# HMCL-UNIST/AD_MPC

Measured on AMD Instinct MI355X. Metric: MPC solves/sec (N=20, nx=7, nu=2, fp64), higher is better.
Workload: dtype f64

## Files before the change

ad_mpc_amd/csrc/admpc_fused20.hip:

```cpp
#include <hip/hip_runtime.h>
#include <type_traits>
#include <stdint.h>
#include <math.h>
#include "../../include/admpc.h"

namespace {

typedef double d4 __attribute__((ext_vector_type(4)));

#include "cond_common.h"

#if defined(ADMPC_PHASE_TIMERS) || defined(ADMPC_F20_TRACE)
__device__ unsigned long long g_f20_trace[4 * 8192];
#define F20_TRACE_BEGIN() const unsigned long long tr_t0 = clock_real(); unsigned long long tr_t1 = 0
#define F20_TRACE_MID() tr_t1 = clock_real()
#define F20_TRACE_END(inst) do { if (threadIdx.x == 0 && (inst) < 8192) { g_f20_trace[4 * (inst)] = tr_t0; g_f20_trace[4 * (inst) + 1] = clock_real(); g_f20_trace[4 * (inst) + 2] = blockIdx.x; g_f20_trace[4 * (inst) + 3] = tr_t1; } } while (0)
#else
#define F20_TRACE_BEGIN() do { } while (0)
#define F20_TRACE_MID() do { } while (0)
#define F20_TRACE_END(inst) do { } while (0)
#endif
#ifdef ADMPC_PHASE_TIMERS
__device__ unsigned long long g_f20_ticks[16];
#define F20_DECL() unsigned long long ph_acc[8] = {0, 0, 0, 0, 0, 0, 0, 0}; const unsigned long long ph_t0 = clock_ticks(); unsigned long long ph_last = ph_t0
// ... 43 lines not shown
    extern __shared__ double lds_raw[];
    double* const Hp = lds_raw + FusedLds::oH;
    double* const Lp = lds_raw + FusedLds::oL;
    double* const park = lds_raw + FusedLds::oPark;
    double* const cb = lds_raw + FusedLds::oCb;
    double* const invd = cb + 64;
    double* const sb = invd + 64;
    double* const sb2 = sb + 64;
    double* const JT = lds_raw + FusedLds::oJT;
    double* const GT = lds_raw + FusedLds::oGT;
    double* const bl = lds_raw + FusedLds::oBl;
    double* const dqC = lds_raw + FusedLds::oDqC;
    double* const gam = lds_raw + FusedLds::oGam;
    double* const dqE = lds_raw + FusedLds::oDqC;
    double* const dus = lds_raw + FusedLds::oGam;
    double* const slot = slotbuf + (size_t)blockIdx.x * FusedLds::NTRI;
    constexpr int slot_aux = 16;
#define PK_DL   park[0 * 64 + lane]
#define PK_DUU  park[1 * 64 + lane]
#define PK_G0   park[2 * 64 + lane]
#define PK_DDL  park[3 * 64 + lane]
#define PK_DDU  park[4 * 64 + lane]

    const Dense40Lds W{Hp, Lp, cb, invd};
    auto factorise = [&](const double dbar_, const double sodd_, const int lz_) __attribute__((always_inline)) {
        dense40_factorise(W, lz_, dbar_, sodd_, lz_, [&](double (&)[n]) __attribute__((always_inline)) {
            if (lz_ < n) Lp[lz_ * (lz_ + 1) / 2 + lz_] = 0.0;
        });
    };

    F20_DECL();
    bool first_ticket = true;
    int* const sch_incl = reinterpret_cast<int*>(lds_raw + FusedLds::oSch);
    int* const sch_cnt = sch_incl + 64;
    if (cap != 0) {
        LAUNDER_LANE(lane_s);
        const int c = sched[F20_BINS0 + F20_NB - 1 - lane_s];
        sch_cnt[lane_s] = c;
        sch_incl[lane_s] = wave_scan_incl_int(c);
        WSYNC();
    }
    auto ticket_entry_addr = [&](const int t, const int lane_) __attribute__((always_inline)) -> const int* {
        const int incl = sch_incl[lane_], c = sch_cnt[lane_];
        const unsigned long long m = __ballot(incl > t);
        if (m == 0ull) return nullptr;
        const int l = __ffsll((long long)m) - 1;
        const int base = __builtin_amdgcn_readlane(incl - c, l);
        return sched + F20_HDR + (size_t)(F20_NB - 1 - l) * cap + (t - base);
    };
    int next_inst = -2;
    const int grid = (int)gridDim.x;
// ... 265 lines not shown
            const int itmax = cf->ipm_iter_max;
            const bool try_unc = cf->ipm_try_unconstrained != 0.0;
            const double thw = cf->ipm_warm_thr, wrest = cf->ipm_warm_restart;
            const int fbit = (int)cf->ipm_fallback_iter;
            const double inv_nineq = 1.0 / (double)(8 * N + 2 * (N - 1));
            const double ubar_i = ubg[sc];
            const double dl_i = cf->lbu[ji] - ubar_i, duu_i = cf->ubu[ji] - ubar_i;
            double t[4], lam[4], sl = thr, su = thr;
            {
                const double r0[4] = { thr - dl_i, thr + duu_i, thr, thr };
#pragma unroll
                for (int i = 0; i < 4; ++i) { t[i] = r0[i] > thr ? r0[i] : thr; lam[i] = mu0 * rcp_nr(t[i]); }
            }
            double Dt[2] = {1.0, 1.0}, Dlam[2] = {0.0, 0.0}, Ddl = 0.0, Ddu = 0.0, dx6 = 0.0;
            if (dact) {
                const double x6 = xbg[lane * 7 + 6];
                Ddl = cf->lbx_delta - x6; Ddu = cf->ubx_delta - x6;
                dx6 = xh6_own;
                const double r0[2] = { dx6 - Ddl, Ddu - dx6 };
#pragma unroll
                for (int i = 0; i < 2; ++i) { Dt[i] = r0[i] > thr ? r0[i] : thr; Dlam[i] = mu0 * rcp_nr(Dt[i]); }
            }
            PK_DL = dl_i; PK_DUU = duu_i; PK_G0 = g0; PK_DDL = Ddl; PK_DDU = Ddu;
            WSYNC();

            double rmax_prev = 0.0, step = 1e300, stp_local = 1e300, alpha_prev = 1.0;
            bool solved = false, warmed = false, cons = false;
            if (try_unc) {
                int lt = lane; asm volatile("" : "+v"(lt));
                factorise(uact ? Rj : 1.0, 0.0, lt);
                const double xt = dense40_solve(W, uact ? -g0 : 0.0, lt);
                const double duc = uact ? xt : 0.0;
                cb[lane] = duc;
                WSYNC();
                const double du1_stage = lane < N ? cb[2 * lane + 1] : 0.0;
                const double pre = wave_scan_incl<OpSum>(du1_stage);
                const double dx6c = xh6_own + h * (pre - du1_stage);
                const bool ok = (!uact || (duc >= dl_i && duc <= duu_i)) && (!dact || (dx6c >= Ddl && dx6c <= Ddu));
                WSYNC();
                if (__all(ok)) { du = duc; solved = true; }
                else if (thw > 0.0) {
                    warmed = true;
                    du = duc;
                    sl = fmax(dl_i - duc, 0.0) + thw; su = fmax(duc - duu_i, 0.0) + thw;
                    const double r0[4] = { duc + sl - dl_i, su + duu_i - duc, sl, su };
#pragma unroll
                    for (int i = 0; i < 4; ++i) { t[i] = r0[i] > thw ? r0[i] : thw; lam[i] = mu0 * rcp_nr(t[i]); }
                    if (dact) {
                        dx6 = dx6c;
                        const double q0[2] = { dx6 - Ddl, Ddu - dx6 };
#pragma unroll
                        for (int i = 0; i < 2; ++i) { Dt[i] = q0[i] > thw ? q0[i] : thw; Dlam[i] = mu0 * rcp_nr(Dt[i]); }
                    }
                }
// ... 8 lines not shown
                const double q0[2] = { dx6 - PK_DDL, PK_DDU - dx6 };
#pragma unroll
                for (int i = 0; i < 2; ++i) { Dt[i] = dact ? (q0[i] > thr ? q0[i] : thr) : 1.0; Dlam[i] = dact ? mu0 * rcp_nr(Dt[i]) : 0.0; }
                alpha_prev = 1.0; stp_local = 1e300;
            };
        F20_STAMP(4);
            F20_TRACE_MID();
            if (!solved && try_unc) {
                asm volatile("s_waitcnt vmcnt(0)" ::: "memory");
                slot_fetch<FusedLds::NTRI, slot_aux>(Hp, slot, lane);
            }
            if (!solved)
            for (; it < itmax + (cons ? fbit : 0); ++it) {
                if (it == 0) __builtin_amdgcn_s_setprio(1);
                if (it == 2) __builtin_amdgcn_s_setprio(2);
                if (it == 4) __builtin_amdgcn_s_setprio(3);
                int lz = lane;
                asm volatile("" : "+v"(lz));
                const int trz = lz * (lz + 1) / 2;
                const bool uz = lz < n;
                double ru, mu, Dbar, S_i;
                {
                    double musum = 0.0, cmax = 0.0, rmax = 0.0;
                    double G0, G1, G2, G3;
                    {
                        const double i0 = rcp_nr(t[0]), i1 = rcp_nr(t[1]), i2_ = rcp_nr(t[2]), i3 = rcp_nr(t[3]);
                        G0 = lam[0] * i0; G1 = lam[1] * i1; G2 = lam[2] * i2_; G3 = lam[3] * i3;
                    }
#pragma unroll
                    for (int i = 0; i < 4; ++i) { const double rci = t[i] * lam[i]; musum += uact ? rci : 0.0; cmax = fmax(cmax, uact ? rci : 0.0); }
#pragma unroll
                    for (int i = 0; i < 2; ++i) { const double rci = Dt[i] * Dlam[i]; musum += dact ? rci : 0.0; cmax = fmax(cmax, dact ? rci : 0.0); }
                    const double G56 = Dlam[0] * rcp_nr(Dt[0]) + Dlam[1] * rcp_nr(Dt[1]);
                    Dbar = uact ? Rj + G0 * G2 * rcp_nr(G0 + G2) + G1 * G3 * rcp_nr(G1 + G3) : 1.0;
                    cb[lane] = uact ? du : 0.0;
                    const double dlam_pref = wave_scan_incl<OpSum>(dact ? (Dlam[1] - Dlam[0]) : 0.0);
                    sb[lane] = rdlane(dlam_pref, 63) - dlam_pref;
                    const double Ssuf_incl = wave_scan_incl<OpSum>(dact ? G56 : 0.0);
                    sb2[lane] = rdlane(Ssuf_incl, 63) - Ssuf_incl;
                    asm volatile("s_waitcnt vmcnt(0)" ::: "memory");
                    WSYNC();
                    double hdu = 0.0;
                    {
                        double Rd3[3];
#pragma unroll
                        for (int m = 0; m < 3; ++m) Rd3[m] = cb[16 * m + (lane & 15)];
                        double hv[n];
                        sym_row_40(hv, lds_byte_addr(Hp + (uz ? trz : 0)), lds_byte_addr(Hp + (uz ? lz : 0)));
                        static_for<0, n>([&](auto cc) __attribute__((always_inline)) {
                            constexpr int c = decltype(cc)::value;
                            fmac_rowbc_ld<c % 16>(hdu, Rd3[c / 16], hv[c]);
                        });
                    }
                    ru = hdu + Rj * du + PK_G0 - lam[0] + lam[1] + (ji ? h * sb[uact ? ki : 0] : 0.0);
                    S_i = h * h * sb2[uact ? ki : 0];
                    {
                        const double rd0 = du + sl - PK_DL - t[0], rd1 = -du + su + PK_DUU - t[1], rd2 = sl - t[2], rd3 = su - t[3];
                        const double rsl = rho_l - lam[0] - lam[2], rsu = rho_u - lam[1] - lam[3];
                        const double Drd0 = dx6 - PK_DDL - Dt[0], Drd1 = PK_DDU - dx6 - Dt[1];
                        double ra = OpMaxNan::f(fabs(ru), fabs(rsl)); ra = OpMaxNan::f(ra, fabs(rsu));
                        ra = OpMaxNan::f(ra, fabs(rd0)); ra = OpMaxNan::f(ra, fabs(rd1)); ra = OpMaxNan::f(ra, fabs(rd2)); ra = OpMaxNan::f(ra, fabs(rd3));
                        const double rb = OpMaxNan::f(fabs(Drd0), fabs(Drd1));
                        rmax = OpMaxNan::f(uact ? ra : 0.0, dact ? rb : 0.0);
                    }
                    mu = wave_reduce<OpSum>(musum) * inv_nineq;
                    cmax = wave_reduce<OpMax0>(cmax);
                    rmax = wave_reduce<OpMaxNan0>(rmax);
                    step = wave_reduce<OpMax0>(stp_local);
                    if (!(mu == mu) || !(rmax == rmax)) { failed = true; break; }
                    if (cmax <= tol_comp && step <= tol_step &&
                        (rmax <= tol_res || (it > 0 && rmax > 0.1 * rmax_prev && rmax <= ADMPC_IPM_FLOOR_CAP * tol_res))) break;
                    rmax_prev = rmax;
                }
                if (fbit > 0 && !cons && it >= fbit) {
                    cons = true; warmed = false;
                    cold_start();
                    rmax_prev = 0.0;
                    --it;
                    continue;
                }
                factorise(Dbar, (uz && ji) ? S_i : 0.0, lz);
#pragma unroll
                for (int i = 0; i < 4; ++i) asm volatile("" : "+v"(t[i]), "+v"(lam[i]));
#pragma unroll
                for (int i = 0; i < 2; ++i) asm volatile("" : "+v"(Dt[i]), "+v"(Dlam[i]));
                double it_[4], il_[4], rc[4], Dit[2], Dil[2], Drc[2];
#pragma unroll
                for (int i = 0; i < 4; ++i) { it_[i] = rcp_nr(t[i]); il_[i] = rcp_nr(lam[i]); rc[i] = t[i] * lam[i]; }
#pragma unroll
                for (int i = 0; i < 2; ++i) { Dit[i] = rcp_nr(Dt[i]); Dil[i] = rcp_nr(Dlam[i]); Drc[i] = Dt[i] * Dlam[i]; }
                const double G0 = lam[0] * it_[0], G1 = lam[1] * it_[1], G2 = lam[2] * it_[2], G3 = lam[3] * it_[3];
                const double iG02 = rcp_nr(G0 + G2), iG13 = rcp_nr(G1 + G3);
                const double G5 = Dlam[0] * Dit[0], G6 = Dlam[1] * Dit[1];
                const double rd0 = du + sl - PK_DL - t[0], rd1 = -du + su + PK_DUU - t[1], rd2 = sl - t[2], rd3 = su - t[3];
                const double rsl = rho_l - lam[0] - lam[2], rsu = rho_u - lam[1] - lam[3];
                const double Drd0 = dx6 - PK_DDL - Dt[0], Drd1 = PK_DDU - dx6 - Dt[1];

                double mu_aff = 0.0, dsl = 0.0, dsu = 0.0, ddu = 0.0, dt[4], dlam[4], Ddt[2], Ddlam[2];
#pragma unroll 1
                for (int pass = 0; pass < 2; ++pass) {
                    const double c0 = rc[0] * it_[0], c1 = rc[1] * it_[1], c2 = rc[2] * it_[2], c3 = rc[3] * it_[3];
                    const double e1 = rsl + c0 + c2 + G0 * rd0 + G2 * rd2;
                    const double e2 = rsu + c1 + c3 + G1 * rd1 + G3 * rd3;
                    const double etal = c0 + G0 * rd0 - G0 * e1 * iG02;
                    const double etau = -c1 - G1 * rd1 + G1 * e2 * iG13;
                    const double ek = dact ? (Drc[0] * Dit[0] + G5 * Drd0) - (Drc[1] * Dit[1] + G6 * Drd1) : 0.0;
                    const double epref = wave_scan_incl<OpSum>(ek);
                    sb[lane] = rdlane(epref, 63) - epref;
                    WSYNC();
                    double y = uact ? -(ru + etal + etau + (ji ? h * sb[ki] : 0.0)) : 0.0;
                    const double x = dense40_solve(W, y, lz);
                    if (pass == 1) slot_fetch<FusedLds::NTRI, slot_aux>(Hp, slot, lz);
                    ddu = uact ? x : 0.0;
                    cb[lane] = ddu;
                    WSYNC();
                    const double du1_stage = lane < N ? cb[2 * lane + 1] : 0.0;
                    const double pre = wave_scan_incl<OpSum>(du1_stage);
                    const double ddx6 = h * (pre - du1_stage);
                    dsl = -(e1 + G0 * ddu) * iG02;
                    dsu = -(e2 - G1 * ddu) * iG13;
                    dt[0] = ddu + dsl + rd0; dt[1] = -ddu + dsu + rd1; dt[2] = dsl + rd2; dt[3] = dsu + rd3;
                    const double Gs[4] = { G0, G1, G2, G3 };
                    double rr = 0.0;
#pragma unroll
                    for (int i = 0; i < 4; ++i) {
                        dlam[i] = -rc[i] * it_[i] - Gs[i] * dt[i];
                        rr = fmax(rr, uact ? fmax(-dt[i] * it_[i], -dlam[i] * il_[i]) : 0.0);
                    }
                    Ddt[0] = ddx6 + Drd0;  Ddlam[0] = -Drc[0] * Dit[0] - G5 * Ddt[0];
                    Ddt[1] = -ddx6 + Drd1; Ddlam[1] = -Drc[1] * Dit[1] - G6 * Ddt[1];
#pragma unroll
                    for (int i = 0; i < 2; ++i) rr = fmax(rr, dact ? fmax(-Ddt[i] * Dit[i], -Ddlam[i] * Dil[i]) : 0.0);
                    rr = wave_reduce<OpMax0>(rr);
                    const double amax = rr > 1.0 ? rcp_nr(rr) : 1.0;
// ... 225 lines not shown
```

ad_mpc_amd/csrc/dense40.h:

```cpp
#pragma once

__device__ __forceinline__ double rdlane(double v, int l) {
    int lo = __builtin_amdgcn_readlane(__double2loint(v), l);
    int hi = __builtin_amdgcn_readlane(__double2hiint(v), l);
    return __hiloint2double(hi, lo);
}

template <int CTRL, int ROW_MASK>
__device__ __forceinline__ double dpp_mov(double ident, double v) {
    int lo = __builtin_amdgcn_update_dpp(__double2loint(ident), __double2loint(v), CTRL, ROW_MASK, 0xf, false);
    int hi = __builtin_amdgcn_update_dpp(__double2hiint(ident), __double2hiint(v), CTRL, ROW_MASK, 0xf, false);
    return __hiloint2double(hi, lo);
}
template <int CTRL, bool ZF>
__device__ __forceinline__ double dpp_shr(double ident, double v) {
    if constexpr (ZF) {
        int lo = __builtin_amdgcn_update_dpp(0, __double2loint(v), CTRL, 0xf, 0xf, true);
        int hi = __builtin_amdgcn_update_dpp(0, __double2hiint(v), CTRL, 0xf, 0xf, true);
        return __hiloint2double(hi, lo);
    } else return dpp_mov<CTRL, 0xf>(ident, v);
}
struct OpSum { static constexpr bool zf = true; static __device__ __forceinline__ double id() { return 0.0; } static __device__ __forceinline__ double f(double a, double b) { return a + b; } };
struct OpMax { static constexpr bool zf = false; static __device__ __forceinline__ double id() { return -INFINITY; } static __device__ __forceinline__ double f(double a, double b) { return fmax(a, b); } };
struct OpMaxNan { static constexpr bool zf = false; static __device__ __forceinline__ double id() { return -INFINITY; }
// ... 15 lines not shown
#ifdef ADMPC_WSYNC_FENCE_ONLY
#define WSYNC() do { __builtin_amdgcn_fence(__ATOMIC_RELEASE, "wavefront"); __builtin_amdgcn_wave_barrier(); __builtin_amdgcn_fence(__ATOMIC_ACQUIRE, "wavefront"); } while (0)
#else
#define WSYNC() __syncthreads()
#endif

#include "subst_asm.inc"
__device__ __forceinline__ unsigned lds_byte_addr(const double* p) {
    return (unsigned)(size_t)(__attribute__((address_space(3))) const double*)p;
}
__device__ __forceinline__ void fwd_subst_40(double& y, const unsigned row_addr, const unsigned pub_addr) {
    asm volatile(ADMPC_FWD_SUBST_ASM_40 : "+{v[100:101]}"(y) : "{v102}"(row_addr), "{v103}"(pub_addr) : ADMPC_SUBST_CLOBBERS);
}
__device__ __forceinline__ void bwd_subst_40(double& x, const unsigned col_addr, const unsigned pub_addr) {
    asm volatile(ADMPC_BWD_SUBST_ASM_40 : "+{v[100:101]}"(x) : "{v102}"(col_addr), "{v103}"(pub_addr) : ADMPC_SUBST_CLOBBERS);
}

#define RB_OUT(a, o) "=&v"(a[o + 0]), "=&v"(a[o + 1]), "=&v"(a[o + 2]), "=&v"(a[o + 3]), "=&v"(a[o + 4]), "=&v"(a[o + 5]), "=&v"(a[o + 6]), \
                     "=&v"(a[o + 7]), "=&v"(a[o + 8]), "=&v"(a[o + 9]), "=&v"(a[o + 10]), "=&v"(a[o + 11]), "=&v"(a[o + 12]), "=&v"(a[o + 13]), \
                     "=&v"(a[o + 14]), "=&v"(a[o + 15]), "=&v"(a[o + 16]), "=&v"(a[o + 17]), "=&v"(a[o + 18]), "=&v"(a[o + 19])
__device__ __forceinline__ void newton_row_40(double (&a)[40], const unsigned row_addr, const double dbar, const double s_odd) {
    asm volatile(ADMPC_ROWBUILD_ASM_40_A : RB_OUT(a, 0) : "v"(row_addr), "v"(dbar), "v"(s_odd) : "s46", "s47", "memory");
    asm volatile(ADMPC_ROWBUILD_ASM_40_B : RB_OUT(a, 20) : "v"(row_addr), "v"(dbar), "v"(s_odd) : "s46", "s47", "memory");
}

__device__ __forceinline__ void sym_row_40(double (&a)[40], const unsigned row_addr, const unsigned col_addr) {
    asm volatile(ADMPC_SYMROW_ASM_40_A : RB_OUT(a, 0) : "v"(row_addr), "v"(col_addr) : "memory");
    asm volatile(ADMPC_SYMROW_ASM_40_B : RB_OUT(a, 20) : "v"(row_addr), "v"(col_addr) : "memory");
}
template <int NR>
__device__ __forceinline__ void newton_row_40_b(double (&a)[40], const unsigned row_addr, const double dbar, const double s_odd) {
    static_assert(NR == 47 || NR == 54, "generated variants");
    if constexpr (NR == 47) {
        asm volatile(ADMPC_ROWBUILD_ASM_40_A_R47 : RB_OUT(a, 0) : "v"(row_addr), "v"(dbar), "v"(s_odd) : "s46", "s47", "memory");
        asm volatile(ADMPC_ROWBUILD_ASM_40_B_R47 : RB_OUT(a, 20) : "v"(row_addr), "v"(dbar), "v"(s_odd) : "s46", "s47", "memory");
    } else {
        asm volatile(ADMPC_ROWBUILD_ASM_40_A_R54 : RB_OUT(a, 0) : "v"(row_addr), "v"(dbar), "v"(s_odd) : "s46", "s47", "memory");
        asm volatile(ADMPC_ROWBUILD_ASM_40_B_R54 : RB_OUT(a, 20) : "v"(row_addr), "v"(dbar), "v"(s_odd) : "s46", "s47", "memory");
    }
}
template <int NR>
__device__ __forceinline__ void sym_row_40_b(double (&a)[40], const unsigned row_addr, const unsigned col_addr) {
    if constexpr (NR == 47) {
        asm volatile(ADMPC_SYMROW_ASM_40_A_R47 : RB_OUT(a, 0) : "v"(row_addr), "v"(col_addr) : "memory");
        asm volatile(ADMPC_SYMROW_ASM_40_B_R47 : RB_OUT(a, 20) : "v"(row_addr), "v"(col_addr) : "memory");
    } else {
// ... 78 lines not shown
    const auto phi = __builtin_amdgcn_permlane16_swap(hi, hi, false, false);
    if (FIRST_ROW <= 0 || LAST_ROW >= 2) {
        const auto elo = __builtin_amdgcn_permlane32_swap(plo[0], plo[0], false, false);
        const auto ehi = __builtin_amdgcn_permlane32_swap(phi[0], phi[0], false, false);
        if (FIRST_ROW <= 0) R[0] = __hiloint2double((int)ehi[0], (int)elo[0]);
        if (LAST_ROW >= 2) R[2] = __hiloint2double((int)ehi[1], (int)elo[1]);
    }
    if (FIRST_ROW <= 1 && LAST_ROW >= 1) {
        const auto olo = __builtin_amdgcn_permlane32_swap(plo[1], plo[1], false, false);
        const auto ohi = __builtin_amdgcn_permlane32_swap(phi[1], phi[1], false, false);
        R[1] = __hiloint2double((int)ohi[0], (int)olo[0]);
    }
}

__device__ __forceinline__ double rcp_nr(double d) {
    double r = __builtin_amdgcn_rcp(d);
    double e = fma(-d, r, 1.0);
    r = fma(r, e, r);
    e = fma(-d, r, 1.0);
    return fma(r, e, r);
}


struct Dense40Lds { double *Hp, *Lp, *cb, *invd; };
struct Dense40NoFix { __device__ __forceinline__ void operator()(double (&)[40]) const {} };

template <class Fix = Dense40NoFix>
__device__ __forceinline__ void dense40_factorise(const Dense40Lds& W, const int lane, const double dbar_, const double sodd_, const int lz_, const Fix& fix = Fix())
{
    constexpr int n = 40;
    const int trz_ = lz_ * (lz_ + 1) / 2;
    const bool uz_ = lz_ < n;
    double a[n];
    newton_row_40(a, lds_byte_addr(W.Hp + (uz_ ? trz_ : 0)), dbar_, sodd_);
    fix(a);
    const unsigned lrow = lds_byte_addr(W.Lp + (uz_ ? trz_ : 0));
    const unsigned pub_wr = lds_byte_addr(W.cb + lane), pub_rd = lds_byte_addr(W.cb + (lane & 15));
    double* const invd = W.invd;
    auto chain = [&](auto jc, double& nln) __attribute__((always_inline)) {
        constexpr int j = decltype(jc)::value;
        const double dj = rdlane(a[j], j);
        const double dinv = rcp_nr(dj);
        const double lu = a[j] * dinv;
        invd[j] = dinv;
        if constexpr (j + 1 < n) {
            asm volatile("s_bfm_b64 exec, %2, %3\n\tds_write_b64 %0, %1 offset:%4\n\ts_mov_b64 exec, -1"
                         : : "v"(lrow), "v"(lu), "n"(n - 1 - j), "n"(j + 1), "n"(8 * j) : "memory");
            nln = -lu;
        }
    };
    double Rb[2][3] = {{0.0, 0.0, 0.0}, {0.0, 0.0, 0.0}}, nlb[2] = {0.0, 0.0};
    W.cb[lane] = a[0];
#pragma unroll
    for (int m = 0; m < 3; ++m) Rb[0][m] = W.cb[16 * m + (lane & 15)];
    chain(std::integral_constant<int, 0>{}, nlb[0]);
    static_for<0, n - 1>([&](auto jc) __attribute__((always_inline)) {
        constexpr int j = decltype(jc)::value;
        constexpr bool own = (j + 1) / 16 == 2;
        constexpr bool pub = j + 2 < n && (j + 2) / 16 < 2;
        double (&R)[3] = Rb[j & 1];
        double (&Rn)[3] = Rb[(j + 1) & 1];
        double& nl = nlb[j & 1];
        double& nln = nlb[(j + 1) & 1];
        col_head<j + 1, (j + 2) / 16, pub, own>(a[j + 1], R, nl, Rn, pub_wr, pub_rd);
        if constexpr (!pub) Rn[2] = a[j + 1];
        chain(std::integral_constant<int, j + 1>{}, nln);
        constexpr int j4 = ((j + 2 + 3) / 4) * 4 < n ? ((j + 2 + 3) / 4) * 4 : n;
        static_for<j + 2, j4>([&](auto c) __attribute__((always_inline)) {
            constexpr int jj = decltype(c)::value;
            if constexpr (own) fmac_rowbc<jj % 16>(a[jj], R[jj / 16], nl);
            else fmac_rowbc_ld<jj % 16>(a[jj], R[jj / 16], nl);
        });
        static_for<j4 / 4, n / 4>([&](auto c) __attribute__((always_inline)) {
            constexpr int jj = 4 * decltype(c)::value;
            if constexpr (own) fmac_rowbc4<jj % 16>(a[jj], a[jj + 1], a[jj + 2], a[jj + 3], R[jj / 16], nl);
            else fmac_rowbc4_ld<jj % 16>(a[jj], a[jj + 1], a[jj + 2], a[jj + 3], R[jj / 16], nl);
        });
    });
    WSYNC();
}

__device__ __forceinline__ double dense40_solve(const Dense40Lds& W, double y, const int lz_)
{
    const bool uz_ = lz_ < 40;
    const unsigned pub = lds_byte_addr(W.cb + (lz_ & 15));
    fwd_subst_40(y, lds_byte_addr(W.Lp + (uz_ ? lz_ * (lz_ + 1) / 2 : 0)), pub);
    double x = y * W.invd[uz_ ? lz_ : 0];
    bwd_subst_40(x, lds_byte_addr(W.Lp + (uz_ ? lz_ : 0)), pub);
    return x;
}

__device__ __forceinline__ double dense40_symv(const Dense40Lds& W, const int lane, const double v, const int lz_)
{
    constexpr int n = 40;
    const bool uz_ = lz_ < n;
    W.cb[lane] = v;
    WSYNC();
    double Rd3[3];
#pragma unroll
    for (int m = 0; m < 3; ++m) Rd3[m] = W.cb[16 * m + (lane & 15)];
    double hv[n];
    sym_row_40(hv, lds_byte_addr(W.Hp + (uz_ ? lz_ * (lz_ + 1) / 2 : 0)), lds_byte_addr(W.Hp + (uz_ ? lz_ : 0)));
    double acc = 0.0;
    static_for<0, n>([&](auto cc) __attribute__((always_inline)) {
        constexpr int c = decltype(cc)::value;
        fmac_rowbc_ld<c % 16>(acc, Rd3[c / 16], hv[c]);
    });
    WSYNC();
    return acc;
}
```

ad_mpc_amd/csrc/gen_subst_asm.py:

```python
#!/usr/bin/env python3
import sys

D = 8
Y, ADDR, RING, SB, SAVE = 100, 102, 104, 40, 46


PUB, RING2, ZB = 103, 120, 136


def _rows(n):
    return [(16 * r, min(16 * r + 15, n - 1)) for r in range((n + 15) // 16)]


def _subst_blocked(n, forward, nrows=None):
    nrows = n if nrows is None else nrows
    assert forward or nrows == n
    rows = _rows(nrows)
    off = (lambda j: 8 * j) if forward else (lambda j: 8 * (j * (j + 1) // 2))
    out = ["s_mov_b64 s[%d:%d], exec" % (SAVE, SAVE + 1)]
    order = rows if forward else rows[::-1]
    inblk = []
    nin = []
    for (r0, r1) in order:
        js = [j for j in range(r0, r1) if j < n] if forward else list(range(r1, r0, -1))
# ... 120 lines not shown
            out.append("ds_read_b64 %%%d, %%%d offset:%d" % (q, CA, 8 * (c * (c + 1) // 2)))
    out.append("s_mov_b64 exec, -1")
    out.append("s_waitcnt lgkmcnt(0)")
    return out


def emit(name, lines):
    body = " \\\n".join('    "%s\\n\\t"' % l for l in lines)
    return "#define %s \\\n%s\n" % (name, body)


def main():
    n = 40
    clob = ", ".join('"v%d"' % r for r in list(range(RING, RING + 2 * D)) + list(range(RING2, RING2 + 2 * D)) + [ZB, ZB + 1]) + ", " + ", ".join('"s%d"' % r for r in (46, 47))
    txt = "// GENERATED by gen_subst_asm.py (n = %d, prefetch depth %d) -- do not edit\n" % (n, D)
    txt += emit("ADMPC_FWD_SUBST_ASM_%d" % n, fwd(n)) + "\n" + emit("ADMPC_BWD_SUBST_ASM_%d" % n, bwd(n)) + "\n"
    txt += emit("ADMPC_ROWBUILD_ASM_%d_A" % n, rowbuild(n, 0, n // 2)) + "\n" + emit("ADMPC_ROWBUILD_ASM_%d_B" % n, rowbuild(n, n // 2, n)) + "\n"
    txt += emit("ADMPC_ROWSTORE_ASM_%d_A" % n, rowstore(n, 0, n // 2)) + "\n" + emit("ADMPC_ROWSTORE_ASM_%d_B" % n, rowstore(n, n // 2, n)) + "\n"
    txt += emit("ADMPC_SYMROW_ASM_%d_A" % n, symrow(n, 0, n // 2)) + "\n" + emit("ADMPC_SYMROW_ASM_%d_B" % n, symrow(n, n // 2, n)) + "\n"
    for nr in (47, 54):
        txt += emit("ADMPC_FWD_SUBST_ASM_%d_R%d" % (n, nr), fwd(n, nr)) + "\n"
        txt += emit("ADMPC_ROWBUILD_ASM_%d_A_R%d" % (n, nr), rowbuild(n, 0, n // 2, nr)) + "\n" + emit("ADMPC_ROWBUILD_ASM_%d_B_R%d" % (n, nr), rowbuild(n, n // 2, n, nr)) + "\n"
        txt += emit("ADMPC_SYMROW_ASM_%d_A_R%d" % (n, nr), symrow(n, 0, n // 2, nr)) + "\n" + emit("ADMPC_SYMROW_ASM_%d_B_R%d" % (n, nr), symrow(n, n // 2, n, nr)) + "\n"
    txt += "#define ADMPC_SUBST_CLOBBERS %s, \"memory\"\n" % clob
    open(sys.argv[1] if len(sys.argv) > 1 else "subst_asm.inc", "w").write(txt)


if __name__ == "__main__":
    main()
```

ad_mpc_amd/csrc/subst_asm.inc:

```
#define ADMPC_FWD_SUBST_ASM_40 \
    "s_mov_b64 s[46:47], exec\n\t" \
    "s_bfm_b64 exec, 16, 0\n\t" \
    "ds_read_b64 v[104:105], v102 offset:0\n\t" \
    "ds_read_b64 v[106:107], v102 offset:8\n\t" \
    "ds_read_b64 v[108:109], v102 offset:16\n\t" \
    "ds_read_b64 v[110:111], v102 offset:24\n\t" \
    "ds_read_b64 v[112:113], v102 offset:32\n\t" \
    "ds_read_b64 v[114:115], v102 offset:40\n\t" \
    "ds_read_b64 v[116:117], v102 offset:48\n\t" \
    "ds_read_b64 v[118:119], v102 offset:56\n\t" \
    "s_waitcnt lgkmcnt(4)\n\t" \
    "v_fmac_f64_dpp v[100:101], v[100:101], -v[104:105] row_newbcast:0 row_mask:0xf bank_mask:0xf\n\t" \
    "ds_read_b64 v[104:105], v102 offset:64\n\t" \
    "s_bfm_b64 exec, 15, 1\n\t" \
    "v_fmac_f64_dpp v[100:101], v[100:101], -v[106:107] row_newbcast:1 row_mask:0xf bank_mask:0xf\n\t" \
    "ds_read_b64 v[106:107], v102 offset:72\n\t" \
    "s_bfm_b64 exec, 14, 2\n\t" \
    "v_fmac_f64_dpp v[100:101], v[100:101], -v[108:109] row_newbcast:2 row_mask:0xf bank_mask:0xf\n\t" \
    "ds_read_b64 v[108:109], v102 offset:80\n\t" \
    "s_bfm_b64 exec, 13, 3\n\t" \
    "v_fmac_f64_dpp v[100:101], v[100:101], -v[110:111] row_newbcast:3 row_mask:0xf bank_mask:0xf\n\t" \
    "ds_read_b64 v[110:111], v102 offset:88\n\t" \
    "s_waitcnt lgkmcnt(4)\n\t" \
    "s_bfm_b64 exec, 12, 4\n\t" \
// ... 2357 lines not shown
    "s_bfm_b64 exec, 19, 35\n\t" \
    "ds_read_b64 %15, %20 offset:280\n\t" \
    "s_bfm_b64 exec, 35, 0\n\t" \
    "ds_read_b64 %15, %21 offset:5040\n\t" \
    "s_bfm_b64 exec, 18, 36\n\t" \
    "ds_read_b64 %16, %20 offset:288\n\t" \
    "s_bfm_b64 exec, 36, 0\n\t" \
    "ds_read_b64 %16, %21 offset:5328\n\t" \
    "s_bfm_b64 exec, 17, 37\n\t" \
    "ds_read_b64 %17, %20 offset:296\n\t" \
    "s_bfm_b64 exec, 37, 0\n\t" \
    "ds_read_b64 %17, %21 offset:5624\n\t" \
    "s_bfm_b64 exec, 16, 38\n\t" \
    "ds_read_b64 %18, %20 offset:304\n\t" \
    "s_bfm_b64 exec, 38, 0\n\t" \
    "ds_read_b64 %18, %21 offset:5928\n\t" \
    "s_bfm_b64 exec, 15, 39\n\t" \
    "ds_read_b64 %19, %20 offset:312\n\t" \
    "s_bfm_b64 exec, 39, 0\n\t" \
    "ds_read_b64 %19, %21 offset:6240\n\t" \
    "s_mov_b64 exec, -1\n\t" \
    "s_waitcnt lgkmcnt(0)\n\t"

#define ADMPC_SUBST_CLOBBERS "v104", "v105", "v106", "v107", "v108", "v109", "v110", "v111", "v112", "v113", "v114", "v115", "v116", "v117", "v118", "v119", "v120", "v121", "v122", "v123", "v124", "v125", "v126", "v127", "v128", "v129", "v130", "v131", "v132", "v133", "v134", "v135", "v136", "v137", "s46", "s47", "memory"
```

Baseline: 24.20 million.

## Fuse forward substitution into Cholesky factorisation via augmented RHS row

Appends the right-hand side as an extra row (lane 40) of the dense 40x40 factorisation, so the forward substitution happens during elimination and only back substitution remains. The RHS residual terms (etal, etau, suffix scan) are now computed before factorisation and written to LDS, and a WSYNC is added before factorise. This removes one serial forward-substitution pass per Newton iteration and per unconstrained try. In exchange it adds extra LDS writes, a new sync, and a generated row-build variant with 41-lane masks.

```diff
diff --git a/ad_mpc_amd/csrc/admpc_fused20.hip b/ad_mpc_amd/csrc/admpc_fused20.hip
--- a/ad_mpc_amd/csrc/admpc_fused20.hip
+++ b/ad_mpc_amd/csrc/admpc_fused20.hip
@@ -89,11 +89,11 @@
 #define PK_DDL  park[3 * 64 + lane]
 #define PK_DDU  park[4 * 64 + lane]
 
-    const Dense40Lds W{Hp, Lp, cb, invd};
+    const Dense40Lds W{Hp, Lp, cb, invd, sb2};
     auto factorise = [&](const double dbar_, const double sodd_, const int lz_) __attribute__((always_inline)) {
         dense40_factorise(W, lz_, dbar_, sodd_, lz_, [&](double (&)[n]) __attribute__((always_inline)) {
             if (lz_ < n) Lp[lz_ * (lz_ + 1) / 2 + lz_] = 0.0;
-        });
+        }, std::true_type{});
     };
 
     F20_DECL();
@@ -405,6 +405,7 @@
                 for (int i = 0; i < 2; ++i) { Dt[i] = r0[i] > thr ? r0[i] : thr; Dlam[i] = mu0 * rcp_nr(Dt[i]); }
             }
             PK_DL = dl_i; PK_DUU = duu_i; PK_G0 = g0; PK_DDL = Ddl; PK_DDU = Ddu;
+            if (try_unc) sb2[lane] = uact ? -g0 : 0.0;
             WSYNC();
 
             double rmax_prev = 0.0, step = 1e300, stp_local = 1e300, alpha_prev = 1.0;
@@ -412,7 +413,7 @@
             if (try_unc) {
                 int lt = lane; asm volatile("" : "+v"(lt));
                 factorise(uact ? Rj : 1.0, 0.0, lt);
-                const double xt = dense40_solve(W, uact ? -g0 : 0.0, lt);
+                const double xt = dense40_solve_back(W, lt);
                 const double duc = uact ? xt : 0.0;
                 cb[lane] = duc;
                 WSYNC();
@@ -467,17 +468,30 @@
                 double ru, mu, Dbar, S_i;
                 {
                     double musum = 0.0, cmax = 0.0, rmax = 0.0;
-                    double G0, G1, G2, G3;
+                    const double i0 = rcp_nr(t[0]), i1 = rcp_nr(t[1]), i2_ = rcp_nr(t[2]), i3 = rcp_nr(t[3]);
+                    const double G0 = lam[0] * i0, G1 = lam[1] * i1, G2 = lam[2] * i2_, G3 = lam[3] * i3;
+#pragma unroll
+                    for (int i = 0; i < 4; ++i) { const double rci = t[i] * lam[i]; musum += uact ? rci : 0.0; cmax = fmax(cmax, uact ? rci : 0.0); }
+#pragma unroll
+                    for (int i = 0; i < 2; ++i) { const double rci = Dt[i] * Dlam[i]; musum += dact ? rci : 0.0; cmax = fmax(cmax, dact ? rci : 0.0); }
+                    const double Di0 = rcp_nr(Dt[0]), Di1 = rcp_nr(Dt[1]);
+                    const double G56 = Dlam[0] * Di0 + Dlam[1] * Di1;
+                    const double iG02 = rcp_nr(G0 + G2), iG13 = rcp_nr(G1 + G3);
+                    Dbar = uact ? Rj + G0 * G2 * iG02 + G1 * G3 * iG13 : 1.0;
+                    double etal, etau;
                     {
-                        const double i0 = rcp_nr(t[0]), i1 = rcp_nr(t[1]), i2_ = rcp_nr(t[2]), i3 = rcp_nr(t[3]);
-                        G0 = lam[0] * i0; G1 = lam[1] * i1; G2 = lam[2] * i2_; G3 = lam[3] * i3;
-                    }
-#pragma unroll
-                    for (int i = 0; i < 4; ++i) { const double rci = t[i] * lam[i]; musum += uact ? rci : 0.0; cmax = fmax(cmax, uact ? rci : 0.0); }
-#pragma unroll
-                    for (int i = 0; i < 2; ++i) { const double rci = Dt[i] * Dlam[i]; musum += dact ? rci : 0.0; cmax = fmax(cmax, dact ? rci : 0.0); }
-                    const double G56 = Dlam[0] * rcp_nr(Dt[0]) + Dlam[1] * rcp_nr(Dt[1]);
-                    Dbar = uact ? Rj + G0 * G2 * rcp_nr(G0 + G2) + G1 * G3 * rcp_nr(G1 + G3) : 1.0;
+                        const double rd0 = du + sl - PK_DL - t[0], rd1 = -du + su + PK_DUU - t[1], rd2 = sl - t[2], rd3 = su - t[3];
+                        const double rsl = rho_l - lam[0] - lam[2], rsu = rho_u - lam[1] - lam[3];
+                        const double c0 = (t[0] * lam[0]) * i0, c1 = (t[1] * lam[1]) * i1, c2 = (t[2] * lam[2]) * i2_, c3 = (t[3] * lam[3]) * i3;
+                        const double e1 = rsl + c0 + c2 + G0 * rd0 + G2 * rd2;
+                        const double e2 = rsu + c1 + c3 + G1 * rd1 + G3 * rd3;
+                        etal = c0 + G0 * rd0 - G0 * e1 * iG02;
+                        etau = -c1 - G1 * rd1 + G1 * e2 * iG13;
+                        const double Drd0 = dx6 - PK_DDL - Dt[0], Drd1 = PK_DDU - dx6 - Dt[1];
+                        const double ek = dact ? ((Dt[0] * Dlam[0]) * Di0 + (Dlam[0] * Di0) * Drd0) - ((Dt[1] * Dlam[1]) * Di1 + (Dlam[1] * Di1) * Drd1) : 0.0;
+                        const double epref = wave_scan_incl<OpSum>(ek);
+                        invd[lane] = rdlane(epref, 63) - epref;
+                    }
                     cb[lane] = uact ? du : 0.0;
                     const double dlam_pref = wave_scan_incl<OpSum>(dact ? (Dlam[1] - Dlam[0]) : 0.0);
                     sb[lane] = rdlane(dlam_pref, 63) - dlam_pref;
@@ -499,6 +513,7 @@
                     }
                     ru = hdu + Rj * du + PK_G0 - lam[0] + lam[1] + (ji ? h * sb[uact ? ki : 0] : 0.0);
                     S_i = h * h * sb2[uact ? ki : 0];
+                    const double esuf = invd[uact ? ki : 0];
                     {
                         const double rd0 = du + sl - PK_DL - t[0], rd1 = -du + su + PK_DUU - t[1], rd2 = sl - t[2], rd3 = su - t[3];
                         const double rsl = rho_l - lam[0] - lam[2], rsu = rho_u - lam[1] - lam[3];
@@ -516,6 +531,7 @@
                     if (cmax <= tol_comp && step <= tol_step &&
                         (rmax <= tol_res || (it > 0 && rmax > 0.1 * rmax_prev && rmax <= ADMPC_IPM_FLOOR_CAP * tol_res))) break;
                     rmax_prev = rmax;
+                    sb2[lane] = uact ? -(ru + etal + etau + (ji ? h * esuf : 0.0)) : 0.0;
                 }
                 if (fbit > 0 && !cons && it >= fbit) {
                     cons = true; warmed = false;
@@ -524,6 +540,7 @@
                     --it;
                     continue;
                 }
+                WSYNC();
                 factorise(Dbar, (uz && ji) ? S_i : 0.0, lz);
 #pragma unroll
                 for (int i = 0; i < 4; ++i) asm volatile("" : "+v"(t[i]), "+v"(lam[i]));
@@ -547,14 +564,19 @@
                     const double c0 = rc[0] * it_[0], c1 = rc[1] * it_[1], c2 = rc[2] * it_[2], c3 = rc[3] * it_[3];
                     const double e1 = rsl + c0 + c2 + G0 * rd0 + G2 * rd2;
                     const double e2 = rsu + c1 + c3 + G1 * rd1 + G3 * rd3;
-                    const double etal = c0 + G0 * rd0 - G0 * e1 * iG02;
-                    const double etau = -c1 - G1 * rd1 + G1 * e2 * iG13;
-                    const double ek = dact ? (Drc[0] * Dit[0] + G5 * Drd0) - (Drc[1] * Dit[1] + G6 * Drd1) : 0.0;
-                    const double epref = wave_scan_incl<OpSum>(ek);
-                    sb[lane] = rdlane(epref, 63) - epref;
-                    WSYNC();
-                    double y = uact ? -(ru + etal + etau + (ji ? h * sb[ki] : 0.0)) : 0.0;
-                    const double x = dense40_solve(W, y, lz);
+                    double z;
+                    if (pass == 0) z = dense40_rhs_row(W, lz);
+                    else {
+                        const double etal = c0 + G0 * rd0 - G0 * e1 * iG02;
+                        const double etau = -c1 - G1 * rd1 + G1 * e2 * iG13;
+                        const double ek = dact ? (Drc[0] * Dit[0] + G5 * Drd0) - (Drc[1] * Dit[1] + G6 * Drd1) : 0.0;
+                        const double epref = wave_scan_incl<OpSum>(ek);
+                        sb[lane] = rdlane(epref, 63) - epref;
+                        WSYNC();
+                        const double y = uact ? -(ru + etal + etau + (ji ? h * sb[ki] : 0.0)) : 0.0;
+                        z = dense40_solve_fwd(W, y, lz);
+                    }
+                    const double x = dense40_solve_bwd(W, z, lz);
                     if (pass == 1) slot_fetch<FusedLds::NTRI, slot_aux>(Hp, slot, lz);
                     ddu = uact ? x : 0.0;
                     cb[lane] = ddu;
diff --git a/ad_mpc_amd/csrc/dense40.h b/ad_mpc_amd/csrc/dense40.h
--- a/ad_mpc_amd/csrc/dense40.h
+++ b/ad_mpc_amd/csrc/dense40.h
@@ -61,6 +61,10 @@
 __device__ __forceinline__ void newton_row_40(double (&a)[40], const unsigned row_addr, const double dbar, const double s_odd) {
     asm volatile(ADMPC_ROWBUILD_ASM_40_A : RB_OUT(a, 0) : "v"(row_addr), "v"(dbar), "v"(s_odd) : "s46", "s47", "memory");
     asm volatile(ADMPC_ROWBUILD_ASM_40_B : RB_OUT(a, 20) : "v"(row_addr), "v"(dbar), "v"(s_odd) : "s46", "s47", "memory");
+}
+__device__ __forceinline__ void newton_row_40_rhs(double (&a)[40], const unsigned row_addr, const double dbar, const double s_odd) {
+    asm volatile(ADMPC_ROWBUILD_ASM_40_A_R41 : RB_OUT(a, 0) : "v"(row_addr), "v"(dbar), "v"(s_odd) : "s46", "s47", "memory");
+    asm volatile(ADMPC_ROWBUILD_ASM_40_B_R41 : RB_OUT(a, 20) : "v"(row_addr), "v"(dbar), "v"(s_odd) : "s46", "s47", "memory");
 }
 
 __device__ __forceinline__ void sym_row_40(double (&a)[40], const unsigned row_addr, const unsigned col_addr) {
@@ -185,19 +189,21 @@
 }
 
 
-struct Dense40Lds { double *Hp, *Lp, *cb, *invd; };
+struct Dense40Lds { double *Hp, *Lp, *cb, *invd; double* rhs = nullptr; };
 struct Dense40NoFix { __device__ __forceinline__ void operator()(double (&)[40]) const {} };
 
-template <class Fix = Dense40NoFix>
-__device__ __forceinline__ void dense40_factorise(const Dense40Lds& W, const int lane, const double dbar_, const double sodd_, const int lz_, const Fix& fix = Fix())
+template <class Fix = Dense40NoFix, bool RHS = false>
+__device__ __forceinline__ void dense40_factorise(const Dense40Lds& W, const int lane, const double dbar_, const double sodd_, const int lz_, const Fix& fix = Fix(),
+                                                  std::integral_constant<bool, RHS> = {})
 {
     constexpr int n = 40;
     const int trz_ = lz_ * (lz_ + 1) / 2;
     const bool uz_ = lz_ < n;
     double a[n];
-    newton_row_40(a, lds_byte_addr(W.Hp + (uz_ ? trz_ : 0)), dbar_, sodd_);
+    if constexpr (RHS) newton_row_40_rhs(a, lz_ == n ? lds_byte_addr(W.rhs) : lds_byte_addr(W.Hp + (uz_ ? trz_ : 0)), dbar_, sodd_);
+    else newton_row_40(a, lds_byte_addr(W.Hp + (uz_ ? trz_ : 0)), dbar_, sodd_);
     fix(a);
-    const unsigned lrow = lds_byte_addr(W.Lp + (uz_ ? trz_ : 0));
+    const unsigned lrow = RHS && lz_ == n ? lds_byte_addr(W.rhs) : lds_byte_addr(W.Lp + (uz_ ? trz_ : 0));
     const unsigned pub_wr = lds_byte_addr(W.cb + lane), pub_rd = lds_byte_addr(W.cb + (lane & 15));
     double* const invd = W.invd;
     auto chain = [&](auto jc, double& nln) __attribute__((always_inline)) {
@@ -206,10 +212,10 @@
         const double dinv = rcp_nr(dj);
         const double lu = a[j] * dinv;
         invd[j] = dinv;
-        if constexpr (j + 1 < n) {
+        if constexpr (j + 1 < n + (RHS ? 1 : 0)) {
             asm volatile("s_bfm_b64 exec, %2, %3\n\tds_write_b64 %0, %1 offset:%4\n\ts_mov_b64 exec, -1"
-                         : : "v"(lrow), "v"(lu), "n"(n - 1 - j), "n"(j + 1), "n"(8 * j) : "memory");
-            nln = -lu;
+                         : : "v"(lrow), "v"(lu), "n"(n - 1 - j + (RHS ? 1 : 0)), "n"(j + 1), "n"(8 * j) : "memory");
+            if constexpr (j + 1 < n) nln = -lu;
         }
     };
     double Rb[2][3] = {{0.0, 0.0, 0.0}, {0.0, 0.0, 0.0}}, nlb[2] = {0.0, 0.0};
@@ -243,14 +249,30 @@
     WSYNC();
 }
 
-__device__ __forceinline__ double dense40_solve(const Dense40Lds& W, double y, const int lz_)
+__device__ __forceinline__ double dense40_solve_fwd(const Dense40Lds& W, double y, const int lz_)
 {
     const bool uz_ = lz_ < 40;
     const unsigned pub = lds_byte_addr(W.cb + (lz_ & 15));
     fwd_subst_40(y, lds_byte_addr(W.Lp + (uz_ ? lz_ * (lz_ + 1) / 2 : 0)), pub);
-    double x = y * W.invd[uz_ ? lz_ : 0];
-    bwd_subst_40(x, lds_byte_addr(W.Lp + (uz_ ? lz_ : 0)), pub);
+    return y * W.invd[uz_ ? lz_ : 0];
+}
+__device__ __forceinline__ double dense40_solve_bwd(const Dense40Lds& W, double x, const int lz_)
+{
+    const bool uz_ = lz_ < 40;
+    bwd_subst_40(x, lds_byte_addr(W.Lp + (uz_ ? lz_ : 0)), lds_byte_addr(W.cb + (lz_ & 15)));
     return x;
+}
+__device__ __forceinline__ double dense40_solve(const Dense40Lds& W, double y, const int lz_)
+{
+    return dense40_solve_bwd(W, dense40_solve_fwd(W, y, lz_), lz_);
+}
+__device__ __forceinline__ double dense40_rhs_row(const Dense40Lds& W, const int lz_)
+{
+    return W.rhs[lz_ < 40 ? lz_ : 0];
+}
+__device__ __forceinline__ double dense40_solve_back(const Dense40Lds& W, const int lz_)
+{
+    return dense40_solve_bwd(W, dense40_rhs_row(W, lz_), lz_);
 }
 
 __device__ __forceinline__ double dense40_symv(const Dense40Lds& W, const int lane, const double v, const int lz_)
diff --git a/ad_mpc_amd/csrc/gen_subst_asm.py b/ad_mpc_amd/csrc/gen_subst_asm.py
--- a/ad_mpc_amd/csrc/gen_subst_asm.py
+++ b/ad_mpc_amd/csrc/gen_subst_asm.py
@@ -166,6 +166,7 @@
         txt += emit("ADMPC_FWD_SUBST_ASM_%d_R%d" % (n, nr), fwd(n, nr)) + "\n"
         txt += emit("ADMPC_ROWBUILD_ASM_%d_A_R%d" % (n, nr), rowbuild(n, 0, n // 2, nr)) + "\n" + emit("ADMPC_ROWBUILD_ASM_%d_B_R%d" % (n, nr), rowbuild(n, n // 2, n, nr)) + "\n"
         txt += emit("ADMPC_SYMROW_ASM_%d_A_R%d" % (n, nr), symrow(n, 0, n // 2, nr)) + "\n" + emit("ADMPC_SYMROW_ASM_%d_B_R%d" % (n, nr), symrow(n, n // 2, n, nr)) + "\n"
+    txt += emit("ADMPC_ROWBUILD_ASM_%d_A_R%d" % (n, n + 1), rowbuild(n, 0, n // 2, n + 1)) + "\n" + emit("ADMPC_ROWBUILD_ASM_%d_B_R%d" % (n, n + 1), rowbuild(n, n // 2, n, n + 1)) + "\n"
     txt += "#define ADMPC_SUBST_CLOBBERS %s, \"memory\"\n" % clob
     open(sys.argv[1] if len(sys.argv) > 1 else "subst_asm.inc", "w").write(txt)
 
diff --git a/ad_mpc_amd/csrc/subst_asm.inc b/ad_mpc_amd/csrc/subst_asm.inc
--- a/ad_mpc_amd/csrc/subst_asm.inc
+++ b/ad_mpc_amd/csrc/subst_asm.inc
@@ -2403,4 +2403,236 @@
     "s_mov_b64 exec, -1\n\t" \
     "s_waitcnt lgkmcnt(0)\n\t"
 
+#define ADMPC_ROWBUILD_ASM_40_A_R41 \
+    "s_mov_b64 s[46:47], exec\n\t" \
+    "v_mov_b64 %0, 0\n\t" \
+    "v_mov_b64 %1, 0\n\t" \
+    "v_mov_b64 %2, 0\n\t" \
+    "v_mov_b64 %3, 0\n\t" \
+    "v_mov_b64 %4, 0\n\t" \
+    "v_mov_b64 %5, 0\n\t" \
+    "v_mov_b64 %6, 0\n\t" \
+    "v_mov_b64 %7, 0\n\t" \
+    "v_mov_b64 %8, 0\n\t" \
+    "v_mov_b64 %9, 0\n\t" \
+    "v_mov_b64 %10, 0\n\t" \
+    "v_mov_b64 %11, 0\n\t" \
+    "v_mov_b64 %12, 0\n\t" \
+    "v_mov_b64 %13, 0\n\t" \
+    "v_mov_b64 %14, 0\n\t" \
+    "v_mov_b64 %15, 0\n\t" \
+    "v_mov_b64 %16, 0\n\t" \
+    "v_mov_b64 %17, 0\n\t" \
+    "v_mov_b64 %18, 0\n\t" \
+    "v_mov_b64 %19, 0\n\t" \
+    "s_bfm_b64 exec, 41, 0\n\t" \
+    "ds_read_b64 %0, %20 offset:0\n\t" \
+    "s_bfm_b64 exec, 40, 1\n\t" \
+    "ds_read_b64 %1, %20 offset:8\n\t" \
+    "s_bfm_b64 exec, 39, 2\n\t" \
+    "ds_read_b64 %2, %20 offset:16\n\t" \
+    "s_bfm_b64 exec, 38, 3\n\t" \
+    "ds_read_b64 %3, %20 offset:24\n\t" \
+    "s_bfm_b64 exec, 37, 4\n\t" \
+    "ds_read_b64 %4, %20 offset:32\n\t" \
+    "s_bfm_b64 exec, 36, 5\n\t" \
+    "ds_read_b64 %5, %20 offset:40\n\t" \
+    "s_bfm_b64 exec, 35, 6\n\t" \
+    "ds_read_b64 %6, %20 offset:48\n\t" \
+    "s_bfm_b64 exec, 34, 7\n\t" \
+    "ds_read_b64 %7, %20 offset:56\n\t" \
+    "s_bfm_b64 exec, 33, 8\n\t" \
+    "ds_read_b64 %8, %20 offset:64\n\t" \
+    "s_bfm_b64 exec, 32, 9\n\t" \
+    "ds_read_b64 %9, %20 offset:72\n\t" \
+    "s_bfm_b64 exec, 31, 10\n\t" \
+    "ds_read_b64 %10, %20 offset:80\n\t" \
+    "s_bfm_b64 exec, 30, 11\n\t" \
+    "ds_read_b64 %11, %20 offset:88\n\t" \
+    "s_bfm_b64 exec, 29, 12\n\t" \
+    "ds_read_b64 %12, %20 offset:96\n\t" \
+    "s_bfm_b64 exec, 28, 13\n\t" \
+    "ds_read_b64 %13, %20 offset:104\n\t" \
+    "s_bfm_b64 exec, 27, 14\n\t" \
+    "ds_read_b64 %14, %20 offset:112\n\t" \
+    "s_bfm_b64 exec, 26, 15\n\t" \
+    "ds_read_b64 %15, %20 offset:120\n\t" \
+    "s_bfm_b64 exec, 25, 16\n\t" \
+    "ds_read_b64 %16, %20 offset:128\n\t" \
+    "s_bfm_b64 exec, 24, 17\n\t" \
+    "ds_read_b64 %17, %20 offset:136\n\t" \
+    "s_bfm_b64 exec, 23, 18\n\t" \
+    "ds_read_b64 %18, %20 offset:144\n\t" \
+    "s_bfm_b64 exec, 22, 19\n\t" \
+    "ds_read_b64 %19, %20 offset:152\n\t" \
+    "s_mov_b64 exec, s[46:47]\n\t" \
+    "s_waitcnt lgkmcnt(0)\n\t" \
+    "v_add_f64 %1, %1, %22\n\t" \
+    "v_add_f64 %3, %3, %22\n\t" \
+    "v_add_f64 %5, %5, %22\n\t" \
+    "v_add_f64 %7, %7, %22\n\t" \
+    "v_add_f64 %9, %9, %22\n\t" \
+    "v_add_f64 %11, %11, %22\n\t" \
+    "v_add_f64 %13, %13, %22\n\t" \
+    "v_add_f64 %15, %15, %22\n\t" \
+    "v_add_f64 %17, %17, %22\n\t" \
+    "v_add_f64 %19, %19, %22\n\t" \
+    "s_bfm_b64 exec, 1, 0\n\t" \
+    "v_add_f64 %0, %0, %21\n\t" \
+    "s_bfm_b64 exec, 1, 1\n\t" \
+    "v_add_f64 %1, %1, %21\n\t" \
+    "s_bfm_b64 exec, 1, 2\n\t" \
+    "v_add_f64 %2, %2, %21\n\t" \
+    "s_bfm_b64 exec, 1, 3\n\t" \
+    "v_add_f64 %3, %3, %21\n\t" \
+    "s_bfm_b64 exec, 1, 4\n\t" \
+    "v_add_f64 %4, %4, %21\n\t" \
+    "s_bfm_b64 exec, 1, 5\n\t" \
+    "v_add_f64 %5, %5, %21\n\t" \
+    "s_bfm_b64 exec, 1, 6\n\t" \
+    "v_add_f64 %6, %6, %21\n\t" \
+    "s_bfm_b64 exec, 1, 7\n\t" \
+    "v_add_f64 %7, %7, %21\n\t" \
+    "s_bfm_b64 exec, 1, 8\n\t" \
+    "v_add_f64 %8, %8, %21\n\t" \
+    "s_bfm_b64 exec, 1, 9\n\t" \
+    "v_add_f64 %9, %9, %21\n\t" \
+    "s_bfm_b64 exec, 1, 10\n\t" \
+    "v_add_f64 %10, %10, %21\n\t" \
+    "s_bfm_b64 exec, 1, 11\n\t" \
+    "v_add_f64 %11, %11, %21\n\t" \
+    "s_bfm_b64 exec, 1, 12\n\t" \
+    "v_add_f64 %12, %12, %21\n\t" \
+    "s_bfm_b64 exec, 1, 13\n\t" \
+    "v_add_f64 %13, %13, %21\n\t" \
+    "s_bfm_b64 exec, 1, 14\n\t" \
+    "v_add_f64 %14, %14, %21\n\t" \
+    "s_bfm_b64 exec, 1, 15\n\t" \
+    "v_add_f64 %15, %15, %21\n\t" \
+    "s_bfm_b64 exec, 1, 16\n\t" \
+    "v_add_f64 %16, %16, %21\n\t" \
+    "s_bfm_b64 exec, 1, 17\n\t" \
+    "v_add_f64 %17, %17, %21\n\t" \
+    "s_bfm_b64 exec, 1, 18\n\t" \
+    "v_add_f64 %18, %18, %21\n\t" \
+    "s_bfm_b64 exec, 1, 19\n\t" \
+    "v_add_f64 %19, %19, %21\n\t" \
+    "s_mov_b64 exec, s[46:47]\n\t"
+
+#define ADMPC_ROWBUILD_ASM_40_B_R41 \
+    "s_mov_b64 s[46:47], exec\n\t" \
+    "v_mov_b64 %0, 0\n\t" \
+    "v_mov_b64 %1, 0\n\t" \
+    "v_mov_b64 %2, 0\n\t" \
+    "v_mov_b64 %3, 0\n\t" \
+    "v_mov_b64 %4, 0\n\t" \
+    "v_mov_b64 %5, 0\n\t" \
+    "v_mov_b64 %6, 0\n\t" \
+    "v_mov_b64 %7, 0\n\t" \
+    "v_mov_b64 %8, 0\n\t" \
+    "v_mov_b64 %9, 0\n\t" \
+    "v_mov_b64 %10, 0\n\t" \
+    "v_mov_b64 %11, 0\n\t" \
+    "v_mov_b64 %12, 0\n\t" \
+    "v_mov_b64 %13, 0\n\t" \
+    "v_mov_b64 %14, 0\n\t" \
+    "v_mov_b64 %15, 0\n\t" \
+    "v_mov_b64 %16, 0\n\t" \
+    "v_mov_b64 %17, 0\n\t" \
+    "v_mov_b64 %18, 0\n\t" \
+    "v_mov_b64 %19, 0\n\t" \
+    "s_bfm_b64 exec, 21, 20\n\t" \
+    "ds_read_b64 %0, %20 offset:160\n\t" \
+    "s_bfm_b64 exec, 20, 21\n\t" \
+    "ds_read_b64 %1, %20 offset:168\n\t" \
+    "s_bfm_b64 exec, 19, 22\n\t" \
+    "ds_read_b64 %2, %20 offset:176\n\t" \
+    "s_bfm_b64 exec, 18, 23\n\t" \
+    "ds_read_b64 %3, %20 offset:184\n\t" \
+    "s_bfm_b64 exec, 17, 24\n\t" \
+    "ds_read_b64 %4, %20 offset:192\n\t" \
+    "s_bfm_b64 exec, 16, 25\n\t" \
+    "ds_read_b64 %5, %20 offset:200\n\t" \
+    "s_bfm_b64 exec, 15, 26\n\t" \
+    "ds_read_b64 %6, %20 offset:208\n\t" \
+    "s_bfm_b64 exec, 14, 27\n\t" \
+    "ds_read_b64 %7, %20 offset:216\n\t" \
+    "s_bfm_b64 exec, 13, 28\n\t" \
+    "ds_read_b64 %8, %20 offset:224\n\t" \
+    "s_bfm_b64 exec, 12, 29\n\t" \
+    "ds_read_b64 %9, %20 offset:232\n\t" \
+    "s_bfm_b64 exec, 11, 30\n\t" \
+    "ds_read_b64 %10, %20 offset:240\n\t" \
+    "s_bfm_b64 exec, 10, 31\n\t" \
+    "ds_read_b64 %11, %20 offset:248\n\t" \
+    "s_bfm_b64 exec, 9, 32\n\t" \
+    "ds_read_b64 %12, %20 offset:256\n\t" \
+    "s_bfm_b64 exec, 8, 33\n\t" \
+    "ds_read_b64 %13, %20 offset:264\n\t" \
+    "s_bfm_b64 exec, 7, 34\n\t" \
+    "ds_read_b64 %14, %20 offset:272\n\t" \
+    "s_bfm_b64 exec, 6, 35\n\t" \
+    "ds_read_b64 %15, %20 offset:280\n\t" \
+    "s_bfm_b64 exec, 5, 36\n\t" \
+    "ds_read_b64 %16, %20 offset:288\n\t" \
+    "s_bfm_b64 exec, 4, 37\n\t" \
+    "ds_read_b64 %17, %20 offset:296\n\t" \
+    "s_bfm_b64 exec, 3, 38\n\t" \
+    "ds_read_b64 %18, %20 offset:304\n\t" \
+    "s_bfm_b64 exec, 2, 39\n\t" \
+    "ds_read_b64 %19, %20 offset:312\n\t" \
+    "s_mov_b64 exec, s[46:47]\n\t" \
+    "s_waitcnt lgkmcnt(0)\n\t" \
+    "v_add_f64 %1, %1, %22\n\t" \
+    "v_add_f64 %3, %3, %22\n\t" \
+    "v_add_f64 %5, %5, %22\n\t" \
+    "v_add_f64 %7, %7, %22\n\t" \
+    "v_add_f64 %9, %9, %22\n\t" \
+    "v_add_f64 %11, %11, %22\n\t" \
+    "v_add_f64 %13, %13, %22\n\t" \
+    "v_add_f64 %15, %15, %22\n\t" \
+    "v_add_f64 %17, %17, %22\n\t" \
+    "v_add_f64 %19, %19, %22\n\t" \
+    "s_bfm_b64 exec, 1, 20\n\t" \
+    "v_add_f64 %0, %0, %21\n\t" \
+    "s_bfm_b64 exec, 1, 21\n\t" \
+    "v_add_f64 %1, %1, %21\n\t" \
+    "s_bfm_b64 exec, 1, 22\n\t" \
+    "v_add_f64 %2, %2, %21\n\t" \
+    "s_bfm_b64 exec, 1, 23\n\t" \
+    "v_add_f64 %3, %3, %21\n\t" \
+    "s_bfm_b64 exec, 1, 24\n\t" \
+    "v_add_f64 %4, %4, %21\n\t" \
+    "s_bfm_b64 exec, 1, 25\n\t" \
+    "v_add_f64 %5, %5, %21\n\t" \
+    "s_bfm_b64 exec, 1, 26\n\t" \
+    "v_add_f64 %6, %6, %21\n\t" \
+    "s_bfm_b64 exec, 1, 27\n\t" \
+    "v_add_f64 %7, %7, %21\n\t" \
+    "s_bfm_b64 exec, 1, 28\n\t" \
+    "v_add_f64 %8, %8, %21\n\t" \
+    "s_bfm_b64 exec, 1, 29\n\t" \
+    "v_add_f64 %9, %9, %21\n\t" \
+    "s_bfm_b64 exec, 1, 30\n\t" \
+    "v_add_f64 %10, %10, %21\n\t" \
+    "s_bfm_b64 exec, 1, 31\n\t" \
+    "v_add_f64 %11, %11, %21\n\t" \
+    "s_bfm_b64 exec, 1, 32\n\t" \
+    "v_add_f64 %12, %12, %21\n\t" \
+    "s_bfm_b64 exec, 1, 33\n\t" \
+    "v_add_f64 %13, %13, %21\n\t" \
+    "s_bfm_b64 exec, 1, 34\n\t" \
+    "v_add_f64 %14, %14, %21\n\t" \
+    "s_bfm_b64 exec, 1, 35\n\t" \
+    "v_add_f64 %15, %15, %21\n\t" \
+    "s_bfm_b64 exec, 1, 36\n\t" \
+    "v_add_f64 %16, %16, %21\n\t" \
+    "s_bfm_b64 exec, 1, 37\n\t" \
+    "v_add_f64 %17, %17, %21\n\t" \
+    "s_bfm_b64 exec, 1, 38\n\t" \
+    "v_add_f64 %18, %18, %21\n\t" \
+    "s_bfm_b64 exec, 1, 39\n\t" \
+    "v_add_f64 %19, %19, %21\n\t" \
+    "s_mov_b64 exec, s[46:47]\n\t"
+
 #define ADMPC_SUBST_CLOBBERS "v104", "v105", "v106", "v107", "v108", "v109", "v110", "v111", "v112", "v113", "v114", "v115", "v116", "v117", "v118", "v119", "v120", "v121", "v122", "v123", "v124", "v125", "v126", "v127", "v128", "v129", "v130", "v131", "v132", "v133", "v134", "v135", "v136", "v137", "s46", "s47", "memory"
```

New measurement: 24.66 million (median of 6 runs). 1.9% higher.
